# hanquansanren/DvD

Measured on AMD Instinct MI355X. Metric: documents/sec (50-step DDIM, 288x288 grid), higher is better.
Workload: dtype f16

## Files before the change

dvd_amd/csrc/attention.hip:

```cpp
#include "common.h"
#include "mfma.h"
#include <stdlib.h>

#ifndef DVD_ATTN64_OCC
#define DVD_ATTN64_OCC 2
#endif
#ifndef DVD_ATTN64_ROWSUM
#define DVD_ATTN64_ROWSUM 0
#endif
#ifndef DVD_ATTN_PF
#define DVD_ATTN_PF 4
#endif

namespace dvd {

struct AttnArgs {
  const _Float16* Q;
  const _Float16* K;
  const _Float16* Vt;
  _Float16* O;
  long sQ, sK, sVt, sO;
  int ldq, ldk, ldvt, ldo;
  int heads, batch, tq, tk;
  int kv_div;
  int nqb;
  float c;
  unsigned long long* stamps;
  int xcd_map;
};

__device__ __forceinline__ int kappa(int r) {
  return (r & ~12) | ((r & 4) << 1) | ((r & 8) >> 1);
}

__device__ __forceinline__ float half_swap_max(float x) {
  float a = x, b = x;
  asm volatile("s_nop 1\n\tv_permlane32_swap_b32 %0, %1\n\ts_nop 1" : "+v"(a), "+v"(b));
  return fmaxf(a, b);
}

template <int D>
__global__ void __launch_bounds__(256, (D == 256 ? 1 : 2)) flash_attn_kernel(AttnArgs p) {
  constexpr int KB = 64;
// ... 1218 lines not shown
  }
  const char* kg = uniform_ptr(Kg + (size_t)min(3, nt - 1) * ktile);
  const char* vg = uniform_ptr(Vg + (size_t)min(2, nt - 1) * (KB * 2));
  const int klim = nt - 4, vlim = nt - 3;
  const unsigned kstep = (unsigned)ktile, vstep = KB * 2;
  r64x_prologue_units(kaddr, p.c, m[0], m[1], m[2], m[3]);
  float l[4] = {0.f, 0.f, 0.f, 0.f};
#ifdef DVD_LAB
  if (p.stamps) ts[1] = __builtin_readcyclecounter();
#endif
#define R64X_LOOP_ARGS l[0], l[1], l[2], l[3], kg, vg, nt, kaddr, vrel, koff, voff, p.c, kdst, vdst, kstep, vstep, klim, vlim
#ifdef DVD_LAB
  if constexpr (DBG == 1) r64x_loop_novalu(R64X_LOOP_ARGS);
  else if constexpr (DBG == 2) r64x_loop_nobar(R64X_LOOP_ARGS);
  else if constexpr (DBG == 3) r64x_loop_mfmaonly(R64X_LOOP_ARGS);
  else
#endif
    r64x_loop(R64X_LOOP_ARGS);
#undef R64X_LOOP_ARGS
#ifdef DVD_LAB
  if (p.stamps) ts[2] = __builtin_readcyclecounter();
#endif

  const int lane_e = (int)__builtin_amdgcn_mbcnt_hi(~0u, __builtin_amdgcn_mbcnt_lo(~0u, 0u));
  const int c16e = lane_e & 15, ge = lane_e >> 4;
#pragma unroll
  for (int q = 0; q < 4; ++q) {
    float lt = l[q];
    lt += __shfl_xor(lt, 16);
    lt += __shfl_xor(lt, 32);
// ... 154 lines not shown
#endif

template <int DBG, bool LM>
__global__ void __launch_bounds__(256, 2) __attribute__((amdgpu_num_vgpr(H64X_COMPILER_VGPRS))) flash_attn_h64x_kernel(AttnArgs p) {
  using namespace h64m;
  constexpr int D = 64, KB = 32;
  extern __shared__ __attribute__((aligned(16))) char smem[];
  typedef __attribute__((address_space(3))) void* lptr_t;

  const int nwg = gridDim.x;
  int id = blockIdx.x;
  {
    const int q = nwg / 8, rr = nwg % 8, xcd = id % 8, k = id / 8;
    id = (xcd < rr ? xcd * (q + 1) : rr * (q + 1) + (xcd - rr) * q) + k;
  }
  const int qb = id % p.nqb;
  const int bh = id / p.nqb;
  const int head = bh % p.heads, b = bh / p.heads;
  const int kvb = b / p.kv_div;
  const int tid = threadIdx.x, lane = tid & 63;
  const int wave = __builtin_amdgcn_readfirstlane(tid >> 6);
  const int c16 = lane & 15, g = lane >> 4;

  const _Float16* Qg = p.Q + b * p.sQ + (size_t)head * D;
  const char* Kg = (const char*)(p.K + kvb * p.sK + (size_t)head * D);
  const char* Vg = (const char*)(p.Vt + kvb * p.sVt + (size_t)head * D * p.ldvt);
  {
    const int qrow = qb * 256 + wave * 64 + c16;
    const unsigned rowb = (unsigned)(p.ldq * 2);
    const unsigned q0 = (unsigned)min(qrow, p.tq - 1) * rowb + 16 * g, q1 = (unsigned)min(qrow + 16, p.tq - 1) * rowb + 16 * g;
    const unsigned q2 = (unsigned)min(qrow + 32, p.tq - 1) * rowb + 16 * g, q3 = (unsigned)min(qrow + 48, p.tq - 1) * rowb + 16 * g;
    if constexpr (LM) h64l_load_q((const _Float16*)uniform_ptr((const char*)Qg), q0, q1, q2, q3, p.c);
    else h64x_load_q((const _Float16*)uniform_ptr((const char*)Qg), q0, q1, q2, q3, p.c);
  }
  unsigned koff, voff;
  {
    const int i = 8 * (wave & 1) + (lane >> 3), kb2 = wave >> 1;
    const int key = 8 * (i >> 2) + 4 * kb2 + (i & 3);
    koff = (unsigned)key * (unsigned)(p.ldk * 2) + (unsigned)(((lane & 7) ^ ((i >> 1) & 7)) * 16);
    voff = (unsigned)(16 * wave + (lane >> 2)) * (unsigned)(p.ldvt * 2) + (unsigned)(((lane & 3) ^ ((0u - (unsigned)(lane >> 4)) & 3)) * 16);
  }
// ... 28 lines not shown
  }
  const char* kg = uniform_ptr(Kg + (size_t)min(3, nt - 1) * ktile);
  const char* vg = uniform_ptr(Vg + (size_t)min(2, nt - 1) * (KB * 2));
  const int klim = nt - 4, vlim = nt - 3;
  const unsigned kstep = (unsigned)ktile, vstep = KB * 2;
  if constexpr (LM) h64l_prologue_units(kf0, kf1, m[0], m[1], m[2], m[3]);
  else h64x_prologue_units(kf0, kf1, m[0], m[1], m[2], m[3]);
  float l[4] = {0.f, 0.f, 0.f, 0.f};
#define H64X_TAIL_ARGS kg, vg, nt, kf0, kf1, vrel, koff, voff, kdst, vdst, kstep, vstep, klim, vlim
  if constexpr (LM) {
    const uintx4 ones = {0x3c003c00u, 0x3c003c00u, 0x3c003c00u, 0x3c003c00u};
#ifdef DVD_LAB
    if constexpr (DBG == 1) h64l_loop_novalu(ones, H64X_TAIL_ARGS);
    else if constexpr (DBG == 2) h64l_loop_nobar(ones, H64X_TAIL_ARGS);
    else if constexpr (DBG == 3) h64l_loop_mfmaonly(ones, H64X_TAIL_ARGS);
    else
#endif
      h64l_loop(ones, H64X_TAIL_ARGS);
    l[0] = h64l_read_l<0>(); l[1] = h64l_read_l<1>(); l[2] = h64l_read_l<2>(); l[3] = h64l_read_l<3>();
  } else {
#ifdef DVD_LAB
    if constexpr (DBG == 1) h64x_loop_novalu(l[0], l[1], l[2], l[3], H64X_TAIL_ARGS);
    else if constexpr (DBG == 2) h64x_loop_nobar(l[0], l[1], l[2], l[3], H64X_TAIL_ARGS);
    else if constexpr (DBG == 3) h64x_loop_mfmaonly(l[0], l[1], l[2], l[3], H64X_TAIL_ARGS);
    else
#endif
      h64x_loop(l[0], l[1], l[2], l[3], H64X_TAIL_ARGS);
  }
#undef H64X_TAIL_ARGS

  const int lane_e = (int)__builtin_amdgcn_mbcnt_hi(~0u, __builtin_amdgcn_mbcnt_lo(~0u, 0u));
  const int c16e = lane_e & 15, ge = lane_e >> 4;
#pragma unroll
  for (int q = 0; q < 4; ++q) {
    float lt = l[q];
    if constexpr (!LM) {
      lt += __shfl_xor(lt, 16);
      lt += __shfl_xor(lt, 32);
    }
    const float inv = 1.f / lt;
    const int qglob = qb * 256 + wave * 64 + 16 * q + c16e;
    if (qglob < p.tq) {
      _Float16* op = p.O + b * p.sO + (size_t)qglob * p.ldo + (size_t)head * D + 4 * ge;
      floatx16 x;
      if (q == 0) x = r64m_read_o<0>();
      else if (q == 1) x = r64m_read_o<16>();
      else if (q == 2) x = r64m_read_o<32>();
      else x = r64m_read_o<48>();
#pragma unroll
      for (int db = 0; db < 4; ++db) {
        half4 v;
#pragma unroll
        for (int j = 0; j < 4; ++j) v[j] = (_Float16)(x[4 * db + j] * inv);
        *(half4*)(op + 16 * db) = v;
      }
    }
  }
}
// ... 14 lines not shown
static constexpr int R64_MIN_TQ = 5376;

extern "C" const char* dvd_flash_attn_kernel_name(int head_dim, int tq, int tk) {
  if (head_dim == 32) return "flash_attn_f32_hd32_kernel";
  if (head_dim != 64 && head_dim != 256) return "";
  if (tk % 64 != 0) return head_dim == 256 ? "flash_attn_kernel<256>" : "flash_attn_kernel<64>";
  if (head_dim == 256) return tq >= R64_MIN_TQ ? "flash_attn_r64x_kernel<0>" : "flash_attn_glds_kernel<256, 0>";
  return tq >= R64_MIN_TQ ? "flash_attn_h64x_kernel<0, true>" : "flash_attn_glds_kernel<64, 0>";
}

template <typename KernelT>
static void allow_lds(KernelT kernel, int bytes) {
  (void)hipFuncSetAttribute((const void*)kernel, hipFuncAttributeMaxDynamicSharedMemorySize, bytes);
}

extern "C" int dvd_flash_attn(const dvd_attn_desc* d, void* stream) {
  DVD_REQUIRE(d && d->Q && d->K && d->Vt && d->O, "flash_attn: null pointer");
  DVD_REQUIRE(d->head_dim == 64 || d->head_dim == 256, "flash_attn: head_dim %d not in {64,256}", d->head_dim);
  DVD_REQUIRE(d->heads > 0 && d->batch > 0 && d->tq > 0 && d->tk > 0 && d->kv_batch_div > 0, "flash_attn: bad shape");
  DVD_REQUIRE(d->tk % 8 == 0, "flash_attn: tk=%d must be a multiple of 8", d->tk);
  DVD_REQUIRE(d->ldq % 8 == 0 && d->ldk % 8 == 0 && d->ldvt % 8 == 0 && d->ldo % 4 == 0 &&
                  d->strideQ % 8 == 0 && d->strideK % 8 == 0 && d->strideVt % 8 == 0 && d->strideO % 4 == 0 &&
                  ((uintptr_t)d->Q % 16) == 0 && ((uintptr_t)d->K % 16) == 0 && ((uintptr_t)d->Vt % 16) == 0 &&
                  ((uintptr_t)d->O % 8) == 0,
              "flash_attn: operands must be 16-byte aligned");
  AttnArgs p;
  p.Q = (const _Float16*)d->Q; p.K = (const _Float16*)d->K; p.Vt = (const _Float16*)d->Vt; p.O = (_Float16*)d->O;
  p.sQ = d->strideQ; p.sK = d->strideK; p.sVt = d->strideVt; p.sO = d->strideO;
  p.ldq = d->ldq; p.ldk = d->ldk; p.ldvt = d->ldvt; p.ldo = d->ldo;
  p.heads = d->heads; p.batch = d->batch; p.tq = d->tq; p.tk = d->tk;
  p.kv_div = d->kv_batch_div;
  p.nqb = cdiv(d->tq, 128);
  p.c = d->scale * 1.4426950408889634f;
  p.stamps = nullptr;
  p.xcd_map = 0;
  const long nwg = (long)p.nqb * d->heads * d->batch;
  DVD_REQUIRE(nwg < (1l << 31), "flash_attn: grid too large");
  hipStream_t st = (hipStream_t)stream;
  bool fast = d->tk % 64 == 0;
  bool r64 = d->tq >= R64_MIN_TQ;
  static DeviceOnce attr_done;
  const unsigned long long dev_bit = DeviceOnce::current_bit();
  const bool first_on_device = attr_done.need(dev_bit);
  if (first_on_device) {
    allow_lds(flash_attn_glds_kernel<256, 0>, 2 * (64 * 512 + 256 * 128));
    allow_lds(flash_attn_r64x_kernel<0>, r64p::LDS_BYTES);
    allow_lds(flash_attn_h64x_kernel<0, true>, h64m::LDS_BYTES);
    allow_lds(flash_attn_kernel<256>, 2 * (64 * (2 * 256 + 16) + 256 * (2 * 64 + 16)));
    attr_done.done(dev_bit);
  }
// ... 10 lines not shown
    constexpr int LDS = 2 * (64 * 512 + 256 * 128);
    allow_lds(flash_attn_dsplit_kernel, LDS);
    allow_lds(flash_attn_glds_kernel<256, 1>, LDS);
    allow_lds(flash_attn_glds_kernel<256, 2>, LDS);
    allow_lds(flash_attn_glds_kernel<256, 3>, LDS);
    allow_lds(flash_attn_pipe_kernel<0>, LDS);
    allow_lds(flash_attn_pipe_kernel<1>, LDS);
    allow_lds(flash_attn_r64_kernel<0>, 2 * (32 * 512 + 256 * 64));
    allow_lds(flash_attn_r64_kernel<1>, 2 * (32 * 512 + 256 * 64));
    allow_lds(flash_attn_r64p_kernel<0>, r64p::LDS_BYTES);
    allow_lds(flash_attn_r64p_kernel<1>, r64p::LDS_BYTES);
    allow_lds(flash_attn_r64m_kernel<0>, r64p::LDS_BYTES);
    allow_lds(flash_attn_r64x_kernel<1>, r64p::LDS_BYTES);
    allow_lds(flash_attn_r64x_kernel<2>, r64p::LDS_BYTES);
    allow_lds(flash_attn_r64x_kernel<3>, r64p::LDS_BYTES);
    allow_lds(flash_attn_r64m_kernel<1>, r64p::LDS_BYTES);
    allow_lds(flash_attn_r64m_kernel<2>, r64p::LDS_BYTES);
    allow_lds(flash_attn_r64m_kernel<3>, r64p::LDS_BYTES);
    allow_lds(flash_attn_r64m_kernel<4>, r64p::LDS_BYTES);
    allow_lds(flash_attn_r64m_kernel<5>, r64p::LDS_BYTES);
    allow_lds(flash_attn_r64m_kernel<6>, r64p::LDS_BYTES);
    allow_lds(flash_attn_r64m_kernel<7>, r64p::LDS_BYTES);
  }
  if (fast && d->head_dim == 256) {
    constexpr int LDS = 2 * (64 * 512 + 256 * 128);
    if (getenv("DVD_ATTN_DSPLIT")) {
      flash_attn_dsplit_kernel<<<(unsigned)nwg, 512, LDS, st>>>(p);
      return check_launch("flash_attn(lab dsplit)");
    }
    if (r64 && getenv("DVD_ATTN_R64X_ABL")) {
      p.nqb = cdiv(d->tq, 256);
      const unsigned g = (unsigned)((long)p.nqb * d->heads * d->batch);
      switch (atoi(getenv("DVD_ATTN_R64X_ABL"))) {
        case 1: flash_attn_r64x_kernel<1><<<g, 256, r64p::LDS_BYTES, st>>>(p); break;
        case 2: flash_attn_r64x_kernel<2><<<g, 256, r64p::LDS_BYTES, st>>>(p); break;
        case 3: flash_attn_r64x_kernel<3><<<g, 256, r64p::LDS_BYTES, st>>>(p); break;
        default: flash_attn_r64x_kernel<0><<<g, 256, r64p::LDS_BYTES, st>>>(p);
      }
      return check_launch("flash_attn(lab r64x ablation)");
    }
    if (r64 && (getenv("DVD_ATTN_R64M") || getenv("DVD_ATTN_R64M_ABL"))) {
      p.nqb = cdiv(d->tq, 256);
      const unsigned g = (unsigned)((long)p.nqb * d->heads * d->batch);
      switch (getenv("DVD_ATTN_R64M_ABL") ? atoi(getenv("DVD_ATTN_R64M_ABL")) : 0) {
        case 1: flash_attn_r64m_kernel<1><<<g, 256, r64p::LDS_BYTES, st>>>(p); break;
        case 2: flash_attn_r64m_kernel<2><<<g, 256, r64p::LDS_BYTES, st>>>(p); break;
        case 3: flash_attn_r64m_kernel<3><<<g, 256, r64p::LDS_BYTES, st>>>(p); break;
        case 4: flash_attn_r64m_kernel<4><<<g, 256, r64p::LDS_BYTES, st>>>(p); break;
        case 5: flash_attn_r64m_kernel<5><<<g, 256, r64p::LDS_BYTES, st>>>(p); break;
        case 6: flash_attn_r64m_kernel<6><<<g, 256, r64p::LDS_BYTES, st>>>(p); break;
        case 7: flash_attn_r64m_kernel<7><<<g, 256, r64p::LDS_BYTES, st>>>(p); break;
// ... 25 lines not shown
      else if (bulk) flash_attn_glds_kernel<256, 2><<<(unsigned)nwg, 256, LDS, st>>>(p);
      else flash_attn_glds_kernel<256, 1><<<(unsigned)nwg, 256, LDS, st>>>(p);
      return check_launch("flash_attn(lab glds variant)");
    }
  } else if (fast) {
    constexpr int LDS = 2 * (64 * 128 + 64 * 128);
    if (getenv("DVD_ATTN_H64X") || (r64 && (getenv("DVD_ATTN_H64X_ABL") || getenv("DVD_ATTN_H64X_NOLM")))) {
      p.nqb = cdiv(d->tq, 256);
      const unsigned g = (unsigned)((long)p.nqb * d->heads * d->batch);
      const int abl = getenv("DVD_ATTN_H64X_ABL") ? atoi(getenv("DVD_ATTN_H64X_ABL")) : 0;
      if (getenv("DVD_ATTN_H64X_NOLM")) {
        switch (abl) {
          case 1: flash_attn_h64x_kernel<1, false><<<g, 256, h64m::LDS_BYTES, st>>>(p); break;
          case 2: flash_attn_h64x_kernel<2, false><<<g, 256, h64m::LDS_BYTES, st>>>(p); break;
          case 3: flash_attn_h64x_kernel<3, false><<<g, 256, h64m::LDS_BYTES, st>>>(p); break;
          default: flash_attn_h64x_kernel<0, false><<<g, 256, h64m::LDS_BYTES, st>>>(p);
        }
        return check_launch("flash_attn(lab h64x, row sums on the VALU)");
      }
      switch (abl) {
        case 1: flash_attn_h64x_kernel<1, true><<<g, 256, h64m::LDS_BYTES, st>>>(p); break;
        case 2: flash_attn_h64x_kernel<2, true><<<g, 256, h64m::LDS_BYTES, st>>>(p); break;
        case 3: flash_attn_h64x_kernel<3, true><<<g, 256, h64m::LDS_BYTES, st>>>(p); break;
        default: flash_attn_h64x_kernel<0, true><<<g, 256, h64m::LDS_BYTES, st>>>(p);
      }
      return check_launch("flash_attn(lab h64x)");
    }
    if (getenv("DVD_ATTN_H64M")) {
      p.nqb = cdiv(d->tq, 256);
      const unsigned g = (unsigned)((long)p.nqb * d->heads * d->batch);
      switch (getenv("DVD_ATTN_H64M_ABL") ? atoi(getenv("DVD_ATTN_H64M_ABL")) : 0) {
        case 1: flash_attn_h64m_kernel<1><<<g, 256, h64m::LDS_BYTES, st>>>(p); break;
        case 2: flash_attn_h64m_kernel<2><<<g, 256, h64m::LDS_BYTES, st>>>(p); break;
        case 3: flash_attn_h64m_kernel<3><<<g, 256, h64m::LDS_BYTES, st>>>(p); break;
        default: flash_attn_h64m_kernel<0><<<g, 256, h64m::LDS_BYTES, st>>>(p);
      }
      return check_launch("flash_attn(lab h64m)");
    }
// ... 14 lines not shown
    flash_attn_r64x_kernel<0><<<(unsigned)((long)p.nqb * d->heads * d->batch), 256, r64p::LDS_BYTES, st>>>(p);
  } else if (fast && d->head_dim == 256) {
    flash_attn_glds_kernel<256, 0><<<(unsigned)nwg, 256, 2 * (64 * 512 + 256 * 128), st>>>(p);
  } else if (fast && r64) {
    p.nqb = cdiv(d->tq, 256);
    flash_attn_h64x_kernel<0, true><<<(unsigned)((long)p.nqb * d->heads * d->batch), 256, h64m::LDS_BYTES, st>>>(p);
  } else if (fast) {
    flash_attn_glds_kernel<64, 0><<<(unsigned)nwg, 256, 2 * (64 * 128 + 64 * 128), st>>>(p);
  } else if (d->head_dim == 256) {
    flash_attn_kernel<256><<<(unsigned)nwg, 256, 2 * (64 * (2 * 256 + 16) + 256 * (2 * 64 + 16)), st>>>(p);
  } else {
    flash_attn_kernel<64><<<(unsigned)nwg, 256, 2 * (64 * (2 * 64 + 16) + 64 * (2 * 64 + 16)), st>>>(p);
  }
  return check_launch("flash_attn");
}
```

dvd_amd/csrc/engine.hip:

```cpp
#include <string.h>
#include <algorithm>

#include <string>
#include <vector>

#include "common.h"
#include "gemm_common.h"
#include "mfma.h"

extern "C" {
int dvd_embed_obs_ln(const float*, const float*, const float*, const float*, float*, void*, int, int, void*);
int dvd_layernorm_rows(const float*, int, long, void*, int, long, int, long, int, const float*, const float*,
                       const float*, const float*, int, int, float, void*);
int dvd_build_r_rows(const float*, const float*, const float*, void*, int, int, int, int, int, void*);
int dvd_patch_rows(const float*, long, long, long, long, float*, int, int, int, int, void*);
int dvd_dwconv3x3(const void*, void*, const float*, const float*, int, int, int, void*);
int dvd_colmean(const float*, float*, float*, int, int, int, int, void*);
int dvd_posenc_add(float*, const float*, const float*, const float*, const float*, int, int, int, void*);
int dvd_small_linear(const float*, int, const float*, const float*, float*, int, int, int, int, int, int, int, void*);
int dvd_final_tokens(const float*, const float*, const float*, const float*, const float*, int, int, const float*,
                     const float*, const float*, float*, float*, int, int, void*);
int dvd_im2col3x3(const float*, long, long, long, float*, int, int, int, int, void*);
int dvd_conv3x3_nhwc(const float*, int, const float*, int, const float*, float*, int, int, int, int, void*);
int dvd_maxpool2_nhwc(const float*, float*, int, int, int, void*);
// ... 589 lines not shown
              *g_m = mod + 5 * HID;

  TRY(dvd_embed_obs_ln(x_t, e->F(e->wi.obs_w), e->F(e->wi.obs_b), e->F(e->wi.pos), xtok32, xq16, N, G, stream));
  TRY(dvd_build_r_rows((const float*)e->B(e->bi.feat), init_feat_nchw, init_flow, arows16, RK, N, G, hyp, feat_mode,
                       stream));
  TRY(gemm(F16, (int)NT, HID, RK, 1, arows16, RK, 0, e->H(e->wi.r_w16), RK, 0, nullptr, 0, 0, rtok16, HID, 0, e->F(e->wi.r_b), 0,
           0, e->F(e->wi.pos), T, nullptr, 0, nullptr, 0, 0, stream, nullptr, e->L(e->wi.r_w16)));

  TRY(gemm(F16, (int)NT, HID, HID, 1, xq16, HID, 0, e->H(e->wi.ca_wq16), HID, 0, nullptr, 0, 0, q16, HID, 0, e->F(e->wi.ca_bq),
           0, 0, nullptr, 0, nullptr, 0, nullptr, 0, 0, stream, nullptr, e->L(e->wi.ca_wq16)));
  TRY(gemm(F16, (int)NT, HID, HID, 1, rtok16, HID, 0, e->H(e->wi.ca_wk16), HID, 0, nullptr, 0, 0, kr16, HID, 0,
           e->F(e->wi.ca_bk), 0, 0, nullptr, 0, nullptr, 0, nullptr, 0, 0, stream, nullptr, e->L(e->wi.ca_wk16)));
  TRY(gemm(F16S, HID, T, HID, N, e->H(e->wi.ca_wv16, true), HID, 0, rtok16, HID, (long)T * HID, nullptr, 0, 0, vtr16, T,
           (long)HID * T, e->F(e->wi.ca_bv), 1, 0, nullptr, 0, nullptr, 0, nullptr, 0, 0, stream, e->L(e->wi.ca_wv16, true), nullptr));
  {
    const int kn[3] = {e->bi.kc16, e->bi.km16, e->bi.kl16};
    const int vn[3] = {e->bi.vtc16, e->bi.vtm16, e->bi.vtl16};
    for (int s = 0; s < 3; ++s)
      TRY(attn(64, 6, N, T, T, hyp, q16, HID, (long)T * HID, e->B(kn[s]), HID, (long)T * HID, e->B(vn[s]), T,
               (long)HID * T, att16 + (size_t)s * NT * HID, HID, (long)T * HID, 0.125f, stream));
    TRY(attn(64, 6, N, T, T, 1, q16, HID, (long)T * HID, kr16, HID, (long)T * HID, vtr16, T, (long)HID * T,
             att16 + (size_t)3 * NT * HID, HID, (long)T * HID, 0.125f, stream));
  }
  TRY(gemm(F16, (int)NT, HID, HID, 4, att16, HID, NT * HID, e->H(e->wi.ca_wo16), HID, 0, z, DEC, HID, nullptr, 0, 0,
           e->F(e->wi.ca_bo), 0, 0, nullptr, 0, nullptr, 0, xtok32, HID, 0, stream, nullptr, e->L(e->wi.ca_wo16)));

  if (e->debug_stop == 1) return check_launch("engine_denoise_step(stop 1)");
  TRY(dvd_layernorm_rows(z, DEC, HID, h16, HID, NT * HID, 4, NT, HID, nullptr, nullptr, sh_a, sc_a, 0, (int)NT, 1e-6f,
                         stream));
  TRY(gemm(F16, (int)(4 * NT), 2 * HID, HID, 1, h16, HID, 0, e->H(e->wi.sa_wqk16, true), HID, 0, nullptr, 0, 0, qk16, 2 * HID, 0,
           e->F(e->wi.sa_bqk), 0, 0, nullptr, 0, nullptr, 0, nullptr, 0, 0, stream, nullptr, e->L(e->wi.sa_wqk16, true)));
  TRY(gemm(F16S, HID, T, HID, 4 * N, e->H(e->wi.sa_wv16, true), HID, 0, h16, HID, (long)T * HID, nullptr, 0, 0, vt16, T,
           (long)HID * T, e->F(e->wi.sa_bv), 1, 0, nullptr, 0, nullptr, 0, nullptr, 0, 0, stream, e->L(e->wi.sa_wv16, true), nullptr));
  TRY(attn(64, 6, 4 * N, T, T, 1, qk16, 2 * HID, (long)T * 2 * HID, qk16 + HID, 2 * HID, (long)T * 2 * HID, vt16, T,
           (long)HID * T, att16, HID, (long)T * HID, 0.125f, stream));
  TRY(gemm(F16, (int)NT, HID, HID, 4, att16, HID, NT * HID, e->H(e->wi.sa_wp16), HID, 0, z, DEC, HID, nullptr, 0, 0,
           e->F(e->wi.sa_bp), 0, 0, nullptr, 0, g_a, (int)NT, z, DEC, HID, stream, nullptr, e->L(e->wi.sa_wp16)));
// ... 116 lines not shown
```

dvd_amd/csrc/gen_attn_h64x.py:

```python
#!/usr/bin/env python3
import os
import sys

P0 = 32
FR0 = 48
SBUF = (64, 96)
Q0 = 128
KBYTES, VBYTES = 4096, 4096
S_KG, S_VG, S_TC, S_TMP, S_SEL = 80, 82, 84, 85, 86
SGPR_CLOBBERS = [f"s{i}" for i in range(80, 88)]
THR_BITS = "0x41200000"
ONES_F16X2 = "0x3c003c00"
COMPILER_VGPRS = 32
NEGM0 = 160

MF = "v_mfma_f32_16x16x32_f16"
LM = False
L_SPREAD = os.environ.get("H64X_L_SPREAD") == "1"
PFX = "h64x"
ABL = set()


def vr(lo, n=1):
    return f"v{lo}" if n == 1 else f"v[{lo}:{lo + n - 1}]"
# ... 159 lines not shown
        ring_wait(s, n)
        for qb in range(4):
            d = stile(nxt, kb2, qb)
            s.add(f"{MF} {d}, {frag(n)}, {qreg(qb, ks)}, {vr(NEGM0 + 4 * qb, 4) if ks == 0 else d}")
            if qb == 0:
                a, off = read_for_step(n + 3, slot)
                s.add(f"ds_read_b128 {frag(n + 3)}, %[{a}] offset:{off}")
                if f == 1:
                    dma_m0(s, "k", slot)
            if qb == 2 and f == 1:
                dma(s, "k")
                advance(s, "k")
            emit_gap(s, gaps[4 * f + qb])
    s.add("s_waitcnt vmcnt(1)")
    s.add("s_barrier")
    seq = max_chain(nxt)
    seq.append(f"s_cbranch_vccnz .Lh64x_stub{var}_%=")
    seq.append(f".Lh64x_back{var}_%=:")
    order = [("pk", 0), ("pk", 1), ("e", 0), ("e", 1), ("pk", 2), ("e", 2), ("e", 3), ("pk", 3), ("e", 4), ("e", 5), ("pk", 4),
             ("e", 6), ("e", 7), ("pk", 5), ("e", 8), ("e", 9), ("pk", 6), ("e", 10), ("e", 11), ("pk", 7), ("e", 12), ("e", 13),
             ("e", 14), ("e", 15)] + [("pk", k) for k in range(8, 16)]
    for kind, i in order:
        if kind == "e":
            seq.append(exp_unit(nxt, i))
    gaps = spread(seq, 20 if LM else 16)
    for g in range(4):
        n = 4 + g
        ring_wait(s, n)
        for qb in range(4):
            s.add(f"{MF} {oreg(qb, g)}, {frag(n)}, {pfrag(qb)}, {oreg(qb, g)}")
            if qb == 0:
                a, off = read_for_step(n + 3, slot)
# ... 104 lines not shown
def prologue_units():
    s = Stmt()
    for f in range(3):
        a, off = kfrag_addr(f, 1)
        s.add(f"ds_read_b128 {frag(f)}, %[{a}] offset:{off}")
    for q in range(4):
        for i in range(4):
            s.add(f"v_sub_f32_e32 v{NEGM0 + 4 * q + i}, 0, %[m{q}]")
    for u in range(32):
        s.add(f"v_sub_f32_e32 v{SBUF[0] + u}, v{SBUF[0] + u}, %[m{u >> 3}]")
    for u in range(16):
        s.add(exp_unit(0, u))
    return s


VARIANTS = [("", ()), ("novalu", ("valu",)), ("nobar", ("bar",)), ("mfmaonly", ("valu", "dma", "read", "wait"))]


def emit_loop(w, sfx):
    w(f"// ---- the key-tile loop{sfx}: six tile variants, the rare rescale block, the drain")
    if LM:
        w(f"__device__ __forceinline__ void {PFX}_loop{sfx}(uintx4 ones, const char* kg, const char* vg, int nt,")
    else:
        w(f"__device__ __forceinline__ void {PFX}_loop{sfx}(float& l0, float& l1, float& l2, float& l3, const char* kg, const char* vg, int nt,")
    w("    unsigned kf0, unsigned kf1, unsigned vrel, unsigned koff, unsigned voff, unsigned kdst, unsigned vdst,")
    w("    unsigned kstep, unsigned vstep, int klim, int vlim) {")
    w("  float a0, a1, a2, a3, t0, t1, t2, t3, t4;")
    w("  asm volatile(")
    w(loop_stmt().text())
    ls = "" if LM else '[l0] "+v"(l0), [l1] "+v"(l1), [l2] "+v"(l2), [l3] "+v"(l3), '
    w(f'      : {ls}[a0] "=&v"(a0), [a1] "=&v"(a1), [a2] "=&v"(a2), [a3] "=&v"(a3),')
# ... 103 lines not shown
```

dvd_amd/csrc/gen_attn_r64x.py:

```python
#!/usr/bin/env python3
import os
import sys

MREG = 28
P0 = 32
FR0 = 48
SBUF = (64, 96)
Q0 = 128
KPIECE = 1056
KBYTES, VBYTES = 16 * KPIECE, 16384
S_KG, S_VG, S_TC, S_TMP, S_SEL, S_C = 80, 82, 84, 85, 86, 90
SGPR_CLOBBERS = [f"s{i}" for i in range(80, 92)]
THR_BITS = "0x41200000"
ONES_F16X2 = "0x3c003c00"
COMPILER_VGPRS = MREG

MF = "v_mfma_f32_16x16x32_f16"
ABL = set()


def vr(lo, n=1):
    return f"v{lo}" if n == 1 else f"v[{lo}:{lo + n - 1}]"


# ... 153 lines not shown
        for qb in range(4):
            d = stile(nxt, kb2, qb)
            s.add(f"{MF} {d}, {frag(n)}, {qreg(qb, ks)}, {'0' if ks == 0 else d}")
            if qb == 0:
                a, off = read_for_step(n + 3, slot)
                s.add(f"ds_read_b128 {frag(n + 3)}, %[{a}] offset:{off}")
                if f in (3, 7, 11, 15):
                    dma_m0(s, "k", slot, f >> 2)
            if qb == 2 and f in (3, 7, 11, 15):
                dma(s, "k", f >> 2)
                if f == 15:
                    advance(s, "k")
            emit_gap(s, gaps[4 * f + qb])
    s.add("s_waitcnt vmcnt(4)")
    s.add("s_barrier")
    seq = max_chain(nxt)
    seq.append(f"s_cbranch_vccnz .Lr64x_stub{var}_%=")
    seq.append(f".Lr64x_back{var}_%=:")
    order = [("pk", 0), ("pk", 1), ("e", 0), ("e", 1), ("pk", 2), ("e", 2), ("e", 3), ("pk", 3), ("e", 4), ("e", 5), ("pk", 4),
             ("e", 6), ("e", 7), ("pk", 5), ("e", 8), ("e", 9), ("pk", 6), ("e", 10), ("e", 11), ("pk", 7), ("e", 12), ("e", 13),
             ("e", 14), ("e", 15)] + [("pk", k) for k in range(8, 16)]
    for kind, i in order:
        if kind == "e":
            seq.append(exp_unit(nxt, i))
        elif i < 8:
            seq.extend(pk_arg(nxt, i))
        else:
            seq.append("\\n\\t".join(pk_arg(nxt, i)))
    gaps = [[] for _ in range(64)]
    pos = 1
    for it in seq:
        gaps[pos].append(it)
# ... 107 lines not shown


def prologue_units():
    s = Stmt()
    for f in range(3):
        s.add(f"ds_read_b128 {frag(f)}, %[kaddr] offset:{KBYTES + (f & 1) * 8 * KPIECE + (f >> 1) * 64}")
    for q in range(4):
        s.add(f"v_mov_b32_e32 v{MREG + q}, %[m{q}]")
    for u in range(32):
        s.add(f"v_fma_f32 v{SBUF[0] + u}, v{SBUF[0] + u}, %[c], -%[m{u >> 3}]")
    for u in range(16):
        s.add(exp_unit(0, u))
    return s


VARIANTS = [("", ()), ("novalu", ("valu",)), ("nobar", ("bar",)), ("mfmaonly", ("valu", "dma", "read", "wait"))]


def emit_loop(w, sfx):
    w(f"// ---- the key-tile loop{sfx}: six tile variants, the rare rescale block, the drain")
    w(f"__device__ __forceinline__ void r64x_loop{sfx}(float& l0, float& l1, float& l2, float& l3, const char* kg, const char* vg, int nt,")
    w("    unsigned kaddr, unsigned vrel, const unsigned (&koff)[4], const unsigned (&voff)[4], float c, unsigned kdst, unsigned vdst,")
    w("    unsigned kstep, unsigned vstep, int klim, int vlim) {")
    w("  float a0, a1, a2, a3, t0, t1, t2, t3, t4;")
    w("  asm volatile(")
    w(loop_stmt().text())
    w('      : [l0] "+v"(l0), [l1] "+v"(l1), [l2] "+v"(l2), [l3] "+v"(l3), [a0] "=&v"(a0), [a1] "=&v"(a1), [a2] "=&v"(a2), [a3] "=&v"(a3),')
    w('        [t0] "=&v"(t0), [t1] "=&v"(t1), [t2] "=&v"(t2), [t3] "=&v"(t3), [t4] "=&v"(t4)')
    w('      : [kg] "s"(kg), [vg] "s"(vg), [nt] "s"(nt), [kaddr] "v"(kaddr), [vrel] "v"(vrel), [koff0] "v"(koff[0]), [koff1] "v"(koff[1]),')
    w('        [koff2] "v"(koff[2]), [koff3] "v"(koff[3]), [voff0] "v"(voff[0]), [voff1] "v"(voff[1]), [voff2] "v"(voff[2]), [voff3] "v"(voff[3]),')
    w('        [c] "s"(c), [kdst] "s"(kdst), [vdst] "s"(vdst), [kstep] "s"(kstep), [vstep] "s"(vstep), [klim] "s"(klim), [vlim] "s"(vlim)')
# ... 65 lines not shown
```

dvd_amd/lib.py:

```python
from __future__ import annotations

import ctypes as C
import os

import torch

_HERE = os.path.dirname(os.path.abspath(__file__))
LIB_PATH = os.path.join(_HERE, "libdvd_hip.so")


class DvdError(RuntimeError):
    pass


def _load():
    if not os.path.exists(LIB_PATH):
        raise DvdError(
            f"{LIB_PATH} is missing: build it with `python -c 'import __graft_entry__ as g; g.build()'` "
            "or `make -C dvd_amd/csrc`.  The DvD engine has no non-HIP fallback.")
    return C.CDLL(LIB_PATH)


_lib = _load()

# ... 43 lines not shown

SIGNATURES = {
    "dvd_grid_sample_bilinear_zeros_ac": [c_void, c_void, c_void, C.c_int, C.c_int, C.c_int, C.c_int, C.c_int,
                                          C.c_int, C.c_int, c_void],
    "dvd_unwarp_f32": [c_void, C.c_int, c_void, c_void, C.c_int, C.c_int, C.c_float, c_void],
    "dvd_unwarp_u8": [c_void, C.c_int, c_void, c_void, C.c_int, C.c_int, C.c_float, c_void],
    "dvd_unwarp_f32_batch": [c_void, C.c_int, c_void, c_void, C.c_int, C.c_int, C.c_int, C.c_float, c_void],
    "dvd_unwarp_u8_batch": [c_void, C.c_int, c_void, c_void, C.c_int, C.c_int, C.c_int, C.c_float, c_void],
    "dvd_unwarp_grid": [c_void, C.c_int, c_void, C.c_int, C.c_int, C.c_float, c_void],
    "dvd_sched_step": [C.POINTER(SchedCoef), c_void, c_void, c_void, c_void, c_void, C.c_int, C.c_int, c_void],
    "dvd_hyp_mean_clamp": [c_void, c_void, C.c_int, C.c_int, C.c_int, c_void],
    "dvd_selftest_mfma": [c_void, c_void, c_void, c_void, c_void],
    "dvd_gemm_nt": [C.POINTER(GemmDesc), c_void],
    "dvd_gemm_kernel_name": [C.POINTER(GemmDesc)],
    "dvd_flash_attn": [C.POINTER(AttnDesc), c_void],
    "dvd_embed_obs_ln": [c_void, c_void, c_void, c_void, c_void, c_void, C.c_int, C.c_int, c_void],
    "dvd_layernorm_rows": [c_void, C.c_int, C.c_long, c_void, C.c_int, C.c_long, C.c_int, C.c_long, C.c_int, c_void,
                           c_void, c_void, c_void, C.c_int, C.c_int, C.c_float, c_void],
    "dvd_build_r_rows": [c_void, c_void, c_void, c_void, C.c_int, C.c_int, C.c_int, C.c_int, C.c_int, c_void],
    "dvd_patch_rows": [c_void, C.c_long, C.c_long, C.c_long, C.c_long, c_void, C.c_int, C.c_int, C.c_int, C.c_int,
                       c_void],
    "dvd_dwconv3x3": [c_void, c_void, c_void, c_void, C.c_int, C.c_int, C.c_int, c_void],
    "dvd_colmean": [c_void, c_void, c_void, C.c_int, C.c_int, C.c_int, C.c_int, c_void],
    "dvd_posenc_add": [c_void, c_void, c_void, c_void, c_void, C.c_int, C.c_int, C.c_int, c_void],
    "dvd_small_linear": [c_void, C.c_int, c_void, c_void, c_void, C.c_int, C.c_int, C.c_int, C.c_int, C.c_int, C.c_int,
                         C.c_int, c_void],
    "dvd_final_tokens": [c_void, c_void, c_void, c_void, c_void, C.c_int, C.c_int, c_void, c_void, c_void, c_void,
                         c_void, C.c_int, C.c_int, c_void],
    "dvd_im2col3x3": [c_void, C.c_long, C.c_long, C.c_long, c_void, C.c_int, C.c_int, C.c_int, C.c_int, c_void],
    "dvd_conv3x3_nhwc": [c_void, C.c_int, c_void, C.c_int, c_void, c_void, C.c_int, C.c_int, C.c_int, C.c_int, c_void],
# ... 100 lines not shown
```

dvd_amd/ops.py:

```python
from __future__ import annotations

import ctypes as C

import numpy as np
import torch

from . import lib
from .lib import ptr, stream_ptr


def _chk(t: torch.Tensor, dtype, name):
    if not t.is_cuda:
        raise lib.DvdError(f"{name}: expected a device tensor (the DvD engine has no CPU path)")
    if t.dtype != dtype or not t.is_contiguous():
        raise lib.DvdError(f"{name}: expected contiguous {dtype}, got {t.dtype} contiguous={t.is_contiguous()}")


def grid_sample(src: torch.Tensor, grid_nchw: torch.Tensor, src_batch_div: int = 1) -> torch.Tensor:
    _chk(src, torch.float32, "src")
    _chk(grid_nchw, torch.float32, "grid")
    n, two, h, w = grid_nchw.shape
    ns, c, hin, win = src.shape
    assert two == 2 and ns * src_batch_div == n
    out = torch.empty((n, c, h, w), dtype=torch.float32, device=src.device)
# ... 141 lines not shown


def flash_attn(q, k, vt, out, heads, head_dim, scale, kv_batch_div=1):
    d = lib.AttnDesc()
    d.head_dim, d.heads, d.batch, d.tq, d.tk = head_dim, heads, q.shape[0], q.shape[1], k.shape[1]
    d.kv_batch_div = kv_batch_div
    d.Q, d.ldq, d.strideQ = q.data_ptr(), q.stride(1), q.stride(0)
    d.K, d.ldk, d.strideK = k.data_ptr(), k.stride(1), k.stride(0)
    d.Vt, d.ldvt, d.strideVt = vt.data_ptr(), vt.stride(1), vt.stride(0)
    d.O, d.ldo, d.strideO = out.data_ptr(), out.stride(1), out.stride(0)
    d.scale = scale
    lib.call("dvd_flash_attn", C.byref(d), stream_ptr())
    return out


def layernorm_rows(x, c, gamma=None, beta=None, shift=None, scale=None, mod_rows=1, eps=1e-6):
    rows = x.shape[0]
    out = torch.empty(rows, c, dtype=torch.float16, device=x.device)
    lib.call("dvd_layernorm_rows", ptr(x), x.stride(0), 0, ptr(out), c, 0, 1, rows, c, ptr(gamma), ptr(beta), ptr(shift),
             ptr(scale), (shift.stride(0) if shift is not None and shift.dim() > 1 else 0), mod_rows, C.c_float(eps),
             stream_ptr())
    return out


def dwconv3x3(x16, w9c, b, n, side):
    out = torch.empty_like(x16)
    lib.call("dvd_dwconv3x3", ptr(x16), ptr(out), ptr(w9c), ptr(b), n, side, x16.shape[-1], stream_ptr())
    return out


# ... 71 lines not shown
```

include/dvd_hip.h:

```cpp
#ifndef DVD_HIP_H
#define DVD_HIP_H

#include <stddef.h>
#include <stdint.h>

#ifdef __cplusplus
extern "C" {
#endif

#define DVD_OK 0
#define DVD_E_ARG (-1)
#define DVD_E_LAUNCH (-2)
#define DVD_E_STATE (-3)

const char* dvd_last_error(void);
int dvd_version(void);


int dvd_grid_sample_bilinear_zeros_ac(const float* src, const float* grid, float* out,
                                      int n, int c, int hin, int win, int h, int w,
                                      int src_batch_div, void* stream);

int dvd_unwarp_f32(const float* flow, int g, const float* src_chw, float* out_hwc,
                   int h, int w, float scale, void* stream);
// ... 38 lines not shown
} dvd_gemm_desc;

int dvd_gemm_nt(const dvd_gemm_desc* desc, void* stream);
const char* dvd_gemm_kernel_name(const dvd_gemm_desc* desc);

typedef struct {
  int head_dim, heads, batch, tq, tk, kv_batch_div;
  const void* Q; int ldq; long strideQ;
  const void* K; int ldk; long strideK;
  const void* Vt; int ldvt; long strideVt;
  void* O; int ldo; long strideO;
  float scale;
} dvd_attn_desc;

int dvd_flash_attn(const dvd_attn_desc* desc, void* stream);
const char* dvd_flash_attn_kernel_name(int head_dim, int tq, int tk);


int dvd_embed_obs_ln(const float* x, const float* w, const float* bias, const float* pos, float* tok32,
                     void* ln16, int n, int g, void* stream);

int dvd_layernorm_rows(const float* in, int ldin, long stride_in, void* out16, int ldout, long stride_out,
                       int batch, long rows, int c, const float* gamma, const float* beta, const float* shift,
                       const float* scale, int ldmod, int mod_rows, float eps, void* stream);

int dvd_build_r_rows(const float* feat_nhwc, const float* init_feat_nchw, const float* flow, void* out16, int ldo,
                     int n, int g, int n_hyp, int mode, void* stream);

int dvd_patch_rows(const float* in, long sn, long sc, long sy, long sx, float* out, int ldo, int n, int c, int g,
                   void* stream);
// ... 90 lines not shown
```

Measured before the change: 0.4923.

## Merge four cross-attention launches sharing Q into one multi-stream kernel launch

```diff
diff --git a/dvd_amd/csrc/attention.hip b/dvd_amd/csrc/attention.hip
--- a/dvd_amd/csrc/attention.hip
+++ b/dvd_amd/csrc/attention.hip
@@ -1,6 +1,7 @@
 #include "common.h"
 #include "mfma.h"
 #include <stdlib.h>
+#include <string.h>
 
 #ifndef DVD_ATTN64_OCC
 #define DVD_ATTN64_OCC 2
@@ -13,6 +14,8 @@
 #endif
 
 namespace dvd {
+
+constexpr int ATTN_MAX_STREAMS = 4;
 
 struct AttnArgs {
   const _Float16* Q;
@@ -27,6 +30,11 @@
   float c;
   unsigned long long* stamps;
   int xcd_map;
+  int nstream;
+  const _Float16* stK[ATTN_MAX_STREAMS];
+  const _Float16* stVt[ATTN_MAX_STREAMS];
+  _Float16* stO[ATTN_MAX_STREAMS];
+  int stkv_div[ATTN_MAX_STREAMS];
 };
 
 __device__ __forceinline__ int kappa(int r) {
@@ -1275,6 +1283,7 @@
   if constexpr (DBG == 1) r64x_loop_novalu(R64X_LOOP_ARGS);
   else if constexpr (DBG == 2) r64x_loop_nobar(R64X_LOOP_ARGS);
   else if constexpr (DBG == 3) r64x_loop_mfmaonly(R64X_LOOP_ARGS);
+  else if constexpr (DBG == 4) r64x_loop_nomax(R64X_LOOP_ARGS);
   else
 #endif
     r64x_loop(R64X_LOOP_ARGS);
@@ -1459,17 +1468,29 @@
     const int q = nwg / 8, rr = nwg % 8, xcd = id % 8, k = id / 8;
     id = (xcd < rr ? xcd * (q + 1) : rr * (q + 1) + (xcd - rr) * q) + k;
   }
+  const _Float16 *Ks = p.K, *Vts = p.Vt;
+  _Float16* Os = p.O;
+  int kv_div = p.kv_div;
+  if (p.nstream > 1) {
+    const int per = p.nqb * p.heads * p.batch;
+    int s = 0;
+    while (s + 1 < p.nstream && id >= per) id -= per, ++s;
+    Ks = s == 0 ? p.stK[0] : s == 1 ? p.stK[1] : s == 2 ? p.stK[2] : p.stK[3];
+    Vts = s == 0 ? p.stVt[0] : s == 1 ? p.stVt[1] : s == 2 ? p.stVt[2] : p.stVt[3];
+    Os = s == 0 ? p.stO[0] : s == 1 ? p.stO[1] : s == 2 ? p.stO[2] : p.stO[3];
+    kv_div = s == 0 ? p.stkv_div[0] : s == 1 ? p.stkv_div[1] : s == 2 ? p.stkv_div[2] : p.stkv_div[3];
+  }
   const int qb = id % p.nqb;
   const int bh = id / p.nqb;
   const int head = bh % p.heads, b = bh / p.heads;
-  const int kvb = b / p.kv_div;
+  const int kvb = b / kv_div;
   const int tid = threadIdx.x, lane = tid & 63;
   const int wave = __builtin_amdgcn_readfirstlane(tid >> 6);
   const int c16 = lane & 15, g = lane >> 4;
 
   const _Float16* Qg = p.Q + b * p.sQ + (size_t)head * D;
-  const char* Kg = (const char*)(p.K + kvb * p.sK + (size_t)head * D);
-  const char* Vg = (const char*)(p.Vt + kvb * p.sVt + (size_t)head * D * p.ldvt);
+  const char* Kg = (const char*)(Ks + kvb * p.sK + (size_t)head * D);
+  const char* Vg = (const char*)(Vts + kvb * p.sVt + (size_t)head * D * p.ldvt);
   {
     const int qrow = qb * 256 + wave * 64 + c16;
     const unsigned rowb = (unsigned)(p.ldq * 2);
@@ -1528,6 +1549,7 @@
     if constexpr (DBG == 1) h64l_loop_novalu(ones, H64X_TAIL_ARGS);
     else if constexpr (DBG == 2) h64l_loop_nobar(ones, H64X_TAIL_ARGS);
     else if constexpr (DBG == 3) h64l_loop_mfmaonly(ones, H64X_TAIL_ARGS);
+    else if constexpr (DBG == 4) h64l_loop_nomax(ones, H64X_TAIL_ARGS);
     else
 #endif
       h64l_loop(ones, H64X_TAIL_ARGS);
@@ -1537,6 +1559,7 @@
     if constexpr (DBG == 1) h64x_loop_novalu(l[0], l[1], l[2], l[3], H64X_TAIL_ARGS);
     else if constexpr (DBG == 2) h64x_loop_nobar(l[0], l[1], l[2], l[3], H64X_TAIL_ARGS);
     else if constexpr (DBG == 3) h64x_loop_mfmaonly(l[0], l[1], l[2], l[3], H64X_TAIL_ARGS);
+    else if constexpr (DBG == 4) h64x_loop_nomax(l[0], l[1], l[2], l[3], H64X_TAIL_ARGS);
     else
 #endif
       h64x_loop(l[0], l[1], l[2], l[3], H64X_TAIL_ARGS);
@@ -1555,7 +1578,7 @@
     const float inv = 1.f / lt;
     const int qglob = qb * 256 + wave * 64 + 16 * q + c16e;
     if (qglob < p.tq) {
-      _Float16* op = p.O + b * p.sO + (size_t)qglob * p.ldo + (size_t)head * D + 4 * ge;
+      _Float16* op = Os + b * p.sO + (size_t)qglob * p.ldo + (size_t)head * D + 4 * ge;
       floatx16 x;
       if (q == 0) x = r64m_read_o<0>();
       else if (q == 1) x = r64m_read_o<16>();
@@ -1600,7 +1623,7 @@
   (void)hipFuncSetAttribute((const void*)kernel, hipFuncAttributeMaxDynamicSharedMemorySize, bytes);
 }
 
-extern "C" int dvd_flash_attn(const dvd_attn_desc* d, void* stream) {
+static int attn_validate(const dvd_attn_desc* d) {
   DVD_REQUIRE(d && d->Q && d->K && d->Vt && d->O, "flash_attn: null pointer");
   DVD_REQUIRE(d->head_dim == 64 || d->head_dim == 256, "flash_attn: head_dim %d not in {64,256}", d->head_dim);
   DVD_REQUIRE(d->heads > 0 && d->batch > 0 && d->tq > 0 && d->tk > 0 && d->kv_batch_div > 0, "flash_attn: bad shape");
@@ -1610,6 +1633,10 @@
                   ((uintptr_t)d->Q % 16) == 0 && ((uintptr_t)d->K % 16) == 0 && ((uintptr_t)d->Vt % 16) == 0 &&
                   ((uintptr_t)d->O % 8) == 0,
               "flash_attn: operands must be 16-byte aligned");
+  return DVD_OK;
+}
+
+static AttnArgs attn_args(const dvd_attn_desc* d) {
   AttnArgs p;
   p.Q = (const _Float16*)d->Q; p.K = (const _Float16*)d->K; p.Vt = (const _Float16*)d->Vt; p.O = (_Float16*)d->O;
   p.sQ = d->strideQ; p.sK = d->strideK; p.sVt = d->strideVt; p.sO = d->strideO;
@@ -1620,6 +1647,16 @@
   p.c = d->scale * 1.4426950408889634f;
   p.stamps = nullptr;
   p.xcd_map = 0;
+  p.nstream = 1;
+  for (int s = 0; s < ATTN_MAX_STREAMS; ++s) {
+    p.stK[s] = p.K; p.stVt[s] = p.Vt; p.stO[s] = p.O; p.stkv_div[s] = p.kv_div;
+  }
+  return p;
+}
+
+extern "C" int dvd_flash_attn(const dvd_attn_desc* d, void* stream) {
+  if (int e = attn_validate(d)) return e;
+  AttnArgs p = attn_args(d);
   const long nwg = (long)p.nqb * d->heads * d->batch;
   DVD_REQUIRE(nwg < (1l << 31), "flash_attn: grid too large");
   hipStream_t st = (hipStream_t)stream;
@@ -1660,6 +1697,7 @@
     allow_lds(flash_attn_r64x_kernel<1>, r64p::LDS_BYTES);
     allow_lds(flash_attn_r64x_kernel<2>, r64p::LDS_BYTES);
     allow_lds(flash_attn_r64x_kernel<3>, r64p::LDS_BYTES);
+    allow_lds(flash_attn_r64x_kernel<4>, r64p::LDS_BYTES);
     allow_lds(flash_attn_r64m_kernel<1>, r64p::LDS_BYTES);
     allow_lds(flash_attn_r64m_kernel<2>, r64p::LDS_BYTES);
     allow_lds(flash_attn_r64m_kernel<3>, r64p::LDS_BYTES);
@@ -1681,6 +1719,7 @@
         case 1: flash_attn_r64x_kernel<1><<<g, 256, r64p::LDS_BYTES, st>>>(p); break;
         case 2: flash_attn_r64x_kernel<2><<<g, 256, r64p::LDS_BYTES, st>>>(p); break;
         case 3: flash_attn_r64x_kernel<3><<<g, 256, r64p::LDS_BYTES, st>>>(p); break;
+        case 4: flash_attn_r64x_kernel<4><<<g, 256, r64p::LDS_BYTES, st>>>(p); break;
         default: flash_attn_r64x_kernel<0><<<g, 256, r64p::LDS_BYTES, st>>>(p);
       }
       return check_launch("flash_attn(lab r64x ablation)");
@@ -1736,6 +1775,7 @@
           case 1: flash_attn_h64x_kernel<1, false><<<g, 256, h64m::LDS_BYTES, st>>>(p); break;
           case 2: flash_attn_h64x_kernel<2, false><<<g, 256, h64m::LDS_BYTES, st>>>(p); break;
           case 3: flash_attn_h64x_kernel<3, false><<<g, 256, h64m::LDS_BYTES, st>>>(p); break;
+          case 4: flash_attn_h64x_kernel<4, false><<<g, 256, h64m::LDS_BYTES, st>>>(p); break;
           default: flash_attn_h64x_kernel<0, false><<<g, 256, h64m::LDS_BYTES, st>>>(p);
         }
         return check_launch("flash_attn(lab h64x, row sums on the VALU)");
@@ -1744,6 +1784,7 @@
         case 1: flash_attn_h64x_kernel<1, true><<<g, 256, h64m::LDS_BYTES, st>>>(p); break;
         case 2: flash_attn_h64x_kernel<2, true><<<g, 256, h64m::LDS_BYTES, st>>>(p); break;
         case 3: flash_attn_h64x_kernel<3, true><<<g, 256, h64m::LDS_BYTES, st>>>(p); break;
+        case 4: flash_attn_h64x_kernel<4, true><<<g, 256, h64m::LDS_BYTES, st>>>(p); break;
         default: flash_attn_h64x_kernel<0, true><<<g, 256, h64m::LDS_BYTES, st>>>(p);
       }
       return check_launch("flash_attn(lab h64x)");
@@ -1788,3 +1829,50 @@
   }
   return check_launch("flash_attn");
 }
+
+#ifdef DVD_LAB
+extern char** environ;
+static bool lab_attn_switch_set() {
+  for (char** e = environ; e && *e; ++e)
+    if (!strncmp(*e, "DVD_ATTN_", 9)) return true;
+  return false;
+}
+#endif
+
+extern "C" int dvd_flash_attn_streams(const dvd_attn_desc* d, int n, void* stream) {
+  DVD_REQUIRE(d && n > 0, "flash_attn_streams: no problems");
+  for (int i = 0; i < n; ++i) {
+    if (int e = attn_validate(&d[i])) return e;
+    const dvd_attn_desc& a = d[0];
+    const dvd_attn_desc& b = d[i];
+    DVD_REQUIRE(b.head_dim == a.head_dim && b.heads == a.heads && b.batch == a.batch && b.tq == a.tq && b.tk == a.tk &&
+                    b.Q == a.Q && b.ldq == a.ldq && b.strideQ == a.strideQ && b.ldk == a.ldk && b.strideK == a.strideK &&
+                    b.ldvt == a.ldvt && b.strideVt == a.strideVt && b.ldo == a.ldo && b.strideO == a.strideO &&
+                    b.scale == a.scale,
+                "flash_attn_streams: problem %d differs from problem 0 in more than K, Vt, O and kv_batch_div", i);
+  }
+  bool merged = d->head_dim == 64 && d->tk % 64 == 0 && d->tq >= R64_MIN_TQ;
+#ifdef DVD_LAB
+  if (lab_attn_switch_set()) merged = false;
+#endif
+  if (!merged) {
+    for (int i = 0; i < n; ++i)
+      if (int e = dvd_flash_attn(&d[i], stream)) return e;
+    return DVD_OK;
+  }
+  for (int i0 = 0; i0 < n; i0 += ATTN_MAX_STREAMS) {
+    const int ns = min(ATTN_MAX_STREAMS, n - i0);
+    AttnArgs p = attn_args(&d[i0]);
+    p.nqb = cdiv(d->tq, 256);
+    p.nstream = ns;
+    for (int s = 0; s < ns; ++s) {
+      p.stK[s] = (const _Float16*)d[i0 + s].K; p.stVt[s] = (const _Float16*)d[i0 + s].Vt; p.stO[s] = (_Float16*)d[i0 + s].O;
+      p.stkv_div[s] = d[i0 + s].kv_batch_div;
+    }
+    const long nwg = (long)p.nqb * d->heads * d->batch * ns;
+    DVD_REQUIRE(nwg < (1l << 31), "flash_attn_streams: grid too large");
+    flash_attn_h64x_kernel<0, true><<<(unsigned)nwg, 256, h64m::LDS_BYTES, (hipStream_t)stream>>>(p);
+    if (int e = check_launch("flash_attn_streams")) return e;
+  }
+  return DVD_OK;
+}
diff --git a/dvd_amd/csrc/engine.hip b/dvd_amd/csrc/engine.hip
--- a/dvd_amd/csrc/engine.hip
+++ b/dvd_amd/csrc/engine.hip
@@ -627,13 +627,19 @@
   TRY(gemm(F16S, HID, T, HID, N, e->H(e->wi.ca_wv16, true), HID, 0, rtok16, HID, (long)T * HID, nullptr, 0, 0, vtr16, T,
            (long)HID * T, e->F(e->wi.ca_bv), 1, 0, nullptr, 0, nullptr, 0, nullptr, 0, 0, stream, e->L(e->wi.ca_wv16, true), nullptr));
   {
-    const int kn[3] = {e->bi.kc16, e->bi.km16, e->bi.kl16};
-    const int vn[3] = {e->bi.vtc16, e->bi.vtm16, e->bi.vtl16};
-    for (int s = 0; s < 3; ++s)
-      TRY(attn(64, 6, N, T, T, hyp, q16, HID, (long)T * HID, e->B(kn[s]), HID, (long)T * HID, e->B(vn[s]), T,
-               (long)HID * T, att16 + (size_t)s * NT * HID, HID, (long)T * HID, 0.125f, stream));
-    TRY(attn(64, 6, N, T, T, 1, q16, HID, (long)T * HID, kr16, HID, (long)T * HID, vtr16, T, (long)HID * T,
-             att16 + (size_t)3 * NT * HID, HID, (long)T * HID, 0.125f, stream));
+    const void* ks[4] = {e->B(e->bi.kc16), e->B(e->bi.km16), e->B(e->bi.kl16), kr16};
+    const void* vts[4] = {e->B(e->bi.vtc16), e->B(e->bi.vtm16), e->B(e->bi.vtl16), vtr16};
+    dvd_attn_desc d[4];
+    memset(d, 0, sizeof(d));
+    for (int s = 0; s < 4; ++s) {
+      d[s].head_dim = 64; d[s].heads = 6; d[s].batch = N; d[s].tq = T; d[s].tk = T; d[s].kv_batch_div = s < 3 ? hyp : 1;
+      d[s].Q = q16; d[s].ldq = HID; d[s].strideQ = (long)T * HID;
+      d[s].K = ks[s]; d[s].ldk = HID; d[s].strideK = (long)T * HID;
+      d[s].Vt = vts[s]; d[s].ldvt = T; d[s].strideVt = (long)HID * T;
+      d[s].O = att16 + (size_t)s * NT * HID; d[s].ldo = HID; d[s].strideO = (long)T * HID;
+      d[s].scale = 0.125f;
+    }
+    TRY(dvd_flash_attn_streams(d, 4, stream));
   }
   TRY(gemm(F16, (int)NT, HID, HID, 4, att16, HID, NT * HID, e->H(e->wi.ca_wo16), HID, 0, z, DEC, HID, nullptr, 0, 0,
            e->F(e->wi.ca_bo), 0, 0, nullptr, 0, nullptr, 0, xtok32, HID, 0, stream, nullptr, e->L(e->wi.ca_wo16)));
diff --git a/dvd_amd/csrc/gen_attn_h64x.py b/dvd_amd/csrc/gen_attn_h64x.py
--- a/dvd_amd/csrc/gen_attn_h64x.py
+++ b/dvd_amd/csrc/gen_attn_h64x.py
@@ -197,8 +197,9 @@
             emit_gap(s, gaps[4 * f + qb])
     s.add("s_waitcnt vmcnt(1)")
     s.add("s_barrier")
-    seq = max_chain(nxt)
-    seq.append(f"s_cbranch_vccnz .Lh64x_stub{var}_%=")
+    seq = [] if "max" in ABL else max_chain(nxt)
+    if "max" not in ABL:
+        seq.append(f"s_cbranch_vccnz .Lh64x_stub{var}_%=")
     seq.append(f".Lh64x_back{var}_%=:")
     order = [("pk", 0), ("pk", 1), ("e", 0), ("e", 1), ("pk", 2), ("e", 2), ("e", 3), ("pk", 3), ("e", 4), ("e", 5), ("pk", 4),
              ("e", 6), ("e", 7), ("pk", 5), ("e", 8), ("e", 9), ("pk", 6), ("e", 10), ("e", 11), ("pk", 7), ("e", 12), ("e", 13),
@@ -333,7 +334,8 @@
     return s
 
 
-VARIANTS = [("", ()), ("novalu", ("valu",)), ("nobar", ("bar",)), ("mfmaonly", ("valu", "dma", "read", "wait"))]
+VARIANTS = [("", ()), ("novalu", ("valu",)), ("nobar", ("bar",)), ("mfmaonly", ("valu", "dma", "read", "wait")),
+            ("nomax", ("max",))]
 
 
 def emit_loop(w, sfx):
diff --git a/dvd_amd/csrc/gen_attn_r64x.py b/dvd_amd/csrc/gen_attn_r64x.py
--- a/dvd_amd/csrc/gen_attn_r64x.py
+++ b/dvd_amd/csrc/gen_attn_r64x.py
@@ -191,8 +191,9 @@
             emit_gap(s, gaps[4 * f + qb])
     s.add("s_waitcnt vmcnt(4)")
     s.add("s_barrier")
-    seq = max_chain(nxt)
-    seq.append(f"s_cbranch_vccnz .Lr64x_stub{var}_%=")
+    seq = [] if "max" in ABL else max_chain(nxt)
+    if "max" not in ABL:
+        seq.append(f"s_cbranch_vccnz .Lr64x_stub{var}_%=")
     seq.append(f".Lr64x_back{var}_%=:")
     order = [("pk", 0), ("pk", 1), ("e", 0), ("e", 1), ("pk", 2), ("e", 2), ("e", 3), ("pk", 3), ("e", 4), ("e", 5), ("pk", 4),
              ("e", 6), ("e", 7), ("pk", 5), ("e", 8), ("e", 9), ("pk", 6), ("e", 10), ("e", 11), ("pk", 7), ("e", 12), ("e", 13),
@@ -330,7 +331,8 @@
     return s
 
 
-VARIANTS = [("", ()), ("novalu", ("valu",)), ("nobar", ("bar",)), ("mfmaonly", ("valu", "dma", "read", "wait"))]
+VARIANTS = [("", ()), ("novalu", ("valu",)), ("nobar", ("bar",)), ("mfmaonly", ("valu", "dma", "read", "wait")),
+            ("nomax", ("max",))]
 
 
 def emit_loop(w, sfx):
diff --git a/dvd_amd/lib.py b/dvd_amd/lib.py
--- a/dvd_amd/lib.py
+++ b/dvd_amd/lib.py
@@ -81,6 +81,7 @@
     "dvd_gemm_nt": [C.POINTER(GemmDesc), c_void],
     "dvd_gemm_kernel_name": [C.POINTER(GemmDesc)],
     "dvd_flash_attn": [C.POINTER(AttnDesc), c_void],
+    "dvd_flash_attn_streams": [C.POINTER(AttnDesc), C.c_int, c_void],
     "dvd_embed_obs_ln": [c_void, c_void, c_void, c_void, c_void, c_void, C.c_int, C.c_int, c_void],
     "dvd_layernorm_rows": [c_void, C.c_int, C.c_long, c_void, C.c_int, C.c_long, C.c_int, C.c_long, C.c_int, c_void,
                            c_void, c_void, c_void, C.c_int, C.c_int, C.c_float, c_void],
diff --git a/dvd_amd/ops.py b/dvd_amd/ops.py
--- a/dvd_amd/ops.py
+++ b/dvd_amd/ops.py
@@ -179,6 +179,21 @@
     return out
 
 
+def flash_attn_streams(q, ks, vts, outs, heads, head_dim, scale, kv_batch_divs):
+    n = len(ks)
+    ds = (lib.AttnDesc * n)()
+    for d, k, vt, out, kvd in zip(ds, ks, vts, outs, kv_batch_divs):
+        d.head_dim, d.heads, d.batch, d.tq, d.tk = head_dim, heads, q.shape[0], q.shape[1], k.shape[1]
+        d.kv_batch_div = kvd
+        d.Q, d.ldq, d.strideQ = q.data_ptr(), q.stride(1), q.stride(0)
+        d.K, d.ldk, d.strideK = k.data_ptr(), k.stride(1), k.stride(0)
+        d.Vt, d.ldvt, d.strideVt = vt.data_ptr(), vt.stride(1), vt.stride(0)
+        d.O, d.ldo, d.strideO = out.data_ptr(), out.stride(1), out.stride(0)
+        d.scale = scale
+    lib.call("dvd_flash_attn_streams", ds, n, stream_ptr())
+    return outs
+
+
 def layernorm_rows(x, c, gamma=None, beta=None, shift=None, scale=None, mod_rows=1, eps=1e-6):
     rows = x.shape[0]
     out = torch.empty(rows, c, dtype=torch.float16, device=x.device)
diff --git a/include/dvd_hip.h b/include/dvd_hip.h
--- a/include/dvd_hip.h
+++ b/include/dvd_hip.h
@@ -76,6 +76,7 @@
 } dvd_attn_desc;
 
 int dvd_flash_attn(const dvd_attn_desc* desc, void* stream);
+int dvd_flash_attn_streams(const dvd_attn_desc* descs, int n, void* stream);
 const char* dvd_flash_attn_kernel_name(int head_dim, int tq, int tk);
 
 
```

After: 0.4934 (median of 6 runs). No clear change (+0.2%).
